# thenumbernine/lua-multigrid-poisson

Measured on AMD Instinct MI355X. Metric: V-cycles/sec + finest-smoother achieved HBM GB/s, 3D Poisson, higher is better.
Workload: dtype f32; 1 GPU; BASELINE configs[2]: 3D Poisson 512^3 per GPU, 7-point, RB-GS 2+2, V-cycle, trilinear P, 2x2x2-average R, consistent coarse boundary, per-cycle RMS-update err; parallelism=single GPU, levels=10

## Files before the change

lua-multigrid-poisson_amd/csrc/mgp_kernels.hip:

```cpp
#include "mgp_cell.h"
#include "mgp_zs.h"

#include <cstdio>
#include <cstdlib>
#include <type_traits>
#include <utility>

namespace mgp {
namespace {




template <typename T>
__global__ __launch_bounds__(kBlock) void k_init(T* __restrict__ u, T* __restrict__ f, Geo g, int64_t cx, int64_t cy,
                                                 int64_t cz, int dim3)
{
    const int64_t n = g.P * g.nz;
    for (int64_t s = (int64_t)blockIdx.x * kBlock + threadIdx.x; s < n; s += (int64_t)gridDim.x * kBlock) {
        int i, j;
        int64_t k;
        const bool cell = slot_cell(s, g, i, j, k);
        const double charge = 1e+6, epsilon0 = 1;
        const bool hit = cell && i == cx && j == cy && (!dim3 || g.z0 + k == cz);
// ... 890 lines not shown
            const T a01 = w0 * c01[pe] + w1 * nb01;
            const T a11 = w0 * c11[pe] + w1 * nb11;
            const T b0 = w0 * a00 + w1 * a10;
            const T b1 = w0 * a01 + w1 * a11;
            return w0 * b0 + w1 * b1;
        }
        const bool ox = (o == 0 && I0 + e == 0) || (o == 1 && I0 + e == cx - 1);
        if (!oy && !oz) {
            const T sx = -cl;
            auto nx_ = [&](const T (&cc)[N + 2]) {
                return ox ? (sx == (T)1 ? cc[pe] : sx * cc[pe]) : (o ? cc[e + 2] : cc[e]);
            };
            const T a00 = w0 * c00[pe] + w1 * nx_(c00);
            const T a10 = w0 * c10[pe] + w1 * nx_(c10);
            if (DIM == 2) return w0 * a00 + w1 * a10;
            const T a01 = w0 * c01[pe] + w1 * nx_(c01);
            const T a11 = w0 * c11[pe] + w1 * nx_(c11);
            const T b0 = w0 * a00 + w1 * a10;
            const T b1 = w0 * a01 + w1 * a11;
            return w0 * b0 + w1 * b1;
        }
        auto sv = [&](T val, bool fx, bool fy, bool fz) {
            T s = (T)1;
            if (fx) s = -cl * s;
            if (fy) s = -cl * s;
            if (fz) s = -cl * s;
            return s == (T)1 ? val : s * val;
        };
        auto col = [&](const T (&cc)[N + 2]) { return ox ? cc[pe] : (o ? cc[e + 2] : cc[e]); };
        const T a00 = w0 * c00[pe] + w1 * sv(col(c00), ox, false, false);
        const T a10 = w0 * sv(c10[pe], false, oy, false) + w1 * sv(col(c10), ox, oy, false);
        if (DIM == 2) return w0 * a00 + w1 * a10;
        const T a01 = w0 * sv(c01[pe], false, false, oz) + w1 * sv(col(c01), ox, false, oz);
        const T a11 = w0 * sv(c11[pe], false, oy, oz) + w1 * sv(col(c11), ox, oy, oz);
        const T b0 = w0 * a00 + w1 * a10;
        const T b1 = w0 * a01 + w1 * a11;
        return w0 * b0 + w1 * b1;
    }
};

template <typename T, int DIM, int LINEAR, bool BLACK = false>
__global__ __launch_bounds__(kBlock) void k_prolong_v(T* __restrict__ u, const T* __restrict__ V, Geo g, Geo gc,
                                                      T cl)
{
    constexpr int N = VN<T>::n;
    constexpr int LN = N == 4 ? 2 : 1;
    const int lgpr = gc.lx - LN;
    const int b = xcd_remap(blockIdx.x, gridDim.x);
    const int64_t it = (int64_t)b * kBlock + threadIdx.x;
    const int grp = (int)(it & ((1 << lgpr) - 1));
    const int j = (int)((it >> lgpr) & (g.ny - 1));
    const int64_t k = it >> (lgpr + g.ly);
    if (k >= (DIM == 3 ? (int64_t)g.nz : 1)) return;
    const int I0 = grp * N;
    PvRow<T, N, DIM, LINEAR> pv;
    pv.load(V, gc, j, k, I0);
    const int p = (int)((j + g.z0 + k) & 1);
#pragma unroll
    for (int c = BLACK ? 1 : 0; c < 2; ++c) {
        const int o = c ^ p;
        const int64_t own = k * g.P + c * g.H + (int64_t)j * g.hw + I0;
        Vec<T, N> uv = vload<T, N>(u + own);
#pragma unroll
        for (int e = 0; e < N; ++e) uv.v[e] = uv.v[e] + pv.value(e, o, cl);
        vstore<T, N>(u + own, uv);
    }
}

template <typename T, int DIM, int LINEAR>
__global__ __launch_bounds__(kBlock) void k_post1(T* __restrict__ u, const T* __restrict__ V,
                                                  const T* __restrict__ f, Geo g, Geo gc, Op<T, DIM> op, T clc)
{
    constexpr int N = VN<T>::n;
    constexpr int LN = N == 4 ? 2 : 1;
    const int lgpr = g.lhw - LN;
    const int b = xcd_remap(blockIdx.x, gridDim.x);
    const int64_t it = (int64_t)b * kBlock + threadIdx.x;
    const int grp = (int)(it & ((1 << lgpr) - 1));
    const int j = (int)((it >> lgpr) & (g.ny - 1));
    const int64_t k = it >> (lgpr + g.ly);
    if (k >= g.nz) return;
    const int m0 = grp * N;
    const int64_t gk = g.z0 + k;
    const int orr = (int)((j + gk) & 1);
    auto black_row = [&](int jj, int64_t kk, Vec<T, N>& r) {
        const int64_t gkk = g.z0 + kk;
        if (jj < 0 || jj >= g.ny || (DIM == 3 && (gkk < 0 || gkk >= g.gnz))) {
            r = vzero<T, N>();
            return;
        }
        const int ob = 1 ^ (int)((jj + gkk) & 1);
        r = vload<T, N>(u + kk * g.P + g.H + (int64_t)jj * g.hw + m0);
        PvRow<T, N, DIM, LINEAR> pv;
        pv.load(V, gc, jj, kk, m0);
#pragma unroll
        for (int e = 0; e < N; ++e) r.v[e] = r.v[e] + pv.value(e, ob, clc);
    };
    Vec<T, N> bc, byl, byr, bzl, bzr;
    black_row(j, k, bc);
    black_row(j - 1, k, byl);
    black_row(j + 1, k, byr);
    if (DIM == 3) {
        black_row(j, k - 1, bzl);
        black_row(j, k + 1, bzr);
    }
    const int me = orr == 0 ? m0 - 1 : m0 + N;
    T edge = (T)0;
    if (me >= 0 && me < g.hw) {
        const int i = 2 * me + (orr ^ 1);
        edge = u[k * g.P + g.H + (int64_t)j * g.hw + me] + prolong_value<T, DIM, LINEAR>(V, g, gc, clc, i, j, k);
    }
    const int64_t own = k * g.P + (int64_t)j * g.hw + m0;
    const Vec<T, N> fr = vload<T, N>(f + own);
    const int nbyz = (j == 0) + (j == g.ny - 1) + (DIM == 3 ? (gk == 0) + (gk == g.gnz - 1) : 0);
    Vec<T, N> out;
#pragma unroll
    for (int e = 0; e < N; ++e) {
        const int i = 2 * (m0 + e) + orr;
        const T xl = orr == 0 ? (e == 0 ? edge : bc.v[e - 1]) : bc.v[e];
        const T xr = orr == 0 ? bc.v[e] : (e == N - 1 ? edge : bc.v[e + 1]);
        T s = xl + xr;
        s = s + byl.v[e];
        s = s + byr.v[e];
        if (DIM == 3) {
            s = s + bzl.v[e];
            s = s + bzr.v[e];
        }
        out.v[e] = op.relax(s, fr.v[e], nbyz + (i == 0) + (i == g.nx - 1));
    }
    vstore<T, N>(u + own, out);
}


template <typename T>
struct ZsSplit {
    using S = ZsShape<T, true, true>;
    static_assert(S::XPAIR && S::H == 5 && S::NS3 == 4 && kZsRask, "the split follows k_zs's 64 x 32 PRE layout");
    static constexpr int NTW = S::TC / 64;
    static constexpr int NW = 2 * NTW + 4, NTL = 64 * NW, WMIX = NW - 1;
    static constexpr int MA = S::YT2 - S::YT2S, MB = 2 * S::G;
    static_assert(NTW == 4 && S::NTL == 64 * 7 && S::YT2S == 64 * 6 && S::YT0 == 64 * 5 && MA + MB <= 64, "wave order");
    static constexpr int wave_kind(int w) { return w == WMIX ? 2 : (w < 2 * NTW ? w >= NTW : ((w - 2 * NTW) & 1)); }
    static constexpr int local_wave(int w) { return w < 2 * NTW ? w % NTW : NTW + (w - 2 * NTW) / 2; }
    static constexpr int BT1 = S::YT0 + MB;
    static __device__ __forceinline__ int b_yrow(int t)
    {
        if (t < S::YT0) return S::yrow(t);
        if (t < BT1) return t - S::YT0 < S::G ? S::H - 1 : S::H + S::TY;
        return -1;
    }
    static __device__ __forceinline__ int b_ycol(int t) { return t < S::YT0 ? S::ycol(t) : (t - S::YT0) % S::G; }
    static constexpr int FROWS = S::TY + 2, FSLOT = FROWS * S::HWE;
    static constexpr int OFFFR = (int)(S::lds_bytes / sizeof(T)), OFFFB = OFFFR + 4 * FSLOT;
    static constexpr size_t lds_bytes = (size_t)(OFFFB + 4 * FSLOT) * sizeof(T);
    static_assert(NTL <= 1024 && NW <= 12, "too many waves for 168 VGPRs");
    static_assert(lds_bytes <= 160 * 1024, "LDS");
};

template <typename T, bool ZSRC, bool CLZ>
__device__ __forceinline__ void zs_split_body(const T* __restrict__ src, const T* __restrict__ f, T* __restrict__ dst,
                                              T* __restrict__ R, const Geo& g, const Geo& gc, const Op<T, 3>& op, int zc,
                                              int gz, int patch)
{
    using SP = ZsSplit<T>;
    static_assert(CLZ || (ZsShape<T, true, false>::TX == SP::S::TX && ZsShape<T, true, false>::TY == SP::S::TY &&
                          ZsShape<T, true, false>::N == SP::S::N),
                  "the split's cl != 0 levels run the cl = 0 tile");
    using S = typename SP::S;
    constexpr int N = S::N, H = S::H, HWE = S::HWE, G = S::G, YE = S::YE, SLOT = S::SLOT, TX = S::TX, TY = S::TY,
                  NS3 = S::NS3;
    using VT = Vec<T, N>;
    using PF = ZsPrefetch<T, N>;
    constexpr int PFD = ZS_PFD_PRE, NPF = PFD + 1, UNR = NPF == 3 ? 12 : 4;
    static_assert(PFD >= 1 && PFD <= 3, "prefetch distance 1..3");
    extern __shared__ __align__(16) unsigned char zs_smem[];
    T* const lds = reinterpret_cast<T*>(zs_smem);
    const int tid = threadIdx.x;

    const int tiles_x = g.nx / TX, tiles_y = g.ny / TY;
    const int b = xcd_remap(blockIdx.x, gridDim.x);
    const int tile = b % (tiles_x * tiles_y);
    const int Z0 = (b / (tiles_x * tiles_y)) * zc;
    int tx_, ty_;
    zs_tile_xy(tile, tiles_x, patch, tx_, ty_);
    const int X0 = tx_ * TX, Y0 = ty_ * TY;
    const int hw = g.hw, Hh = (int)g.H;
    const int z0 = (int)g.z0, gnz = (int)g.gnz, cz0 = (int)gc.z0;
    const int64_t P = g.P;
    const int qlo = -gz, qhi = (int)g.nz - 1 + gz;

    const int wv = __builtin_amdgcn_readfirstlane(tid >> 6), lane = tid & 63;
    const int wk = SP::wave_kind(wv), lw = SP::local_wave(wv);
    const bool grp_b = wk == 1 || (wk == 2 && lane >= SP::MA);
    const int lt = wk == 2 ? (grp_b ? S::YT0 + lane - SP::MA : S::YT2S + lane) : 64 * lw + lane;
    const int yr_ = grp_b ? SP::b_yrow(lt) : S::yrow(lt);
    const bool on = yr_ >= 0;
    const int gx = on ? (grp_b ? SP::b_ycol(lt) : S::ycol(lt)) : 0, ye = on ? yr_ : 0;
    const int gy = Y0 - H + ye;
    const int m0 = gx * N;
    ZsCol col;
    col.lrow = ye * HWE + m0;
    col.lym = (ye > 0 ? ye - 1 : ye) * HWE + m0;
    col.lyp = (ye < YE - 1 ? ye + 1 : ye) * HWE + m0;
    col.gm = (X0 - S::HX) / 2 + m0;
    col.x_first = gx == 0;
    col.x_last = gx == G - 1;
    col.lxm = col.x_first ? col.lrow : col.lrow - N;
    col.lxp = col.x_last ? col.lrow : col.lrow + N;
    const bool in_xy = on && gy >= 0 && gy < g.ny && col.gm >= 0 && col.gm < hw;
    col.xin = true;
    const int cgy = gy < 0 ? 0 : (gy >= g.ny ? g.ny - 1 : gy);
    const int cgm = col.gm < 0 ? 0 : (col.gm > hw - N ? hw - N : col.gm);
    const int goff = cgy * hw + cgm;
    const bool tile_xy = on && ye >= H && ye < H + TY && gx >= S::HXG && gx < G - S::HXG;
    const bool frow = on && ye >= H - 1 && ye <= H + TY;
    const int lf = frow ? (ye - (H - 1)) * HWE + m0 : 0;
    auto fslot = [&](int off, int q) { return lds + off + (q & 3) * SP::FSLOT + lf; };
    const int zlo = Z0 - H;
    ZsDiag<T> dz = {};
    if constexpr (!CLZ) {
        const int nby = (gy == 0) + (gy == g.ny - 1);
        dz.db = nby == 0 ? op.dg[0] : (nby == 1 ? op.dg[1] : op.dg[2]);
        dz.yb = nby == 0 ? op.ydg[0] : (nby == 1 ? op.ydg[1] : op.ydg[2]);
        dz.de = nby == 0 ? op.dg[1] : (nby == 1 ? op.dg[2] : op.dg[3]);
        dz.ye = nby == 0 ? op.ydg[1] : (nby == 1 ? op.ydg[2] : op.ydg[3]);
        dz.left = col.gm == 0;
        dz.right = col.gm + N == hw;
    }
    auto nbyz = [&](int q) {
        return CLZ ? 0 : (gy == 0) + (gy == g.ny - 1) + (z0 + q == 0) + (z0 + q == gnz - 1);
    };
    const int p_end = Z0 + zc + 6;
    auto inz = [&](int q) { return z0 + q >= 0 && z0 + q < gnz; };
    auto pcl = [&](int q) { return q < qlo ? qlo : (q > qhi ? qhi : q); };
    auto slot = [&](int off, int ns, int q) { return lds + off + (q & (ns - 1)) * SLOT; };
    const int rowpar = (gy + z0) & 1;
    auto par = [&](int q) { return rowpar ^ (q & 1); };
    const VT vz = vzero<T, N>();

    for (int i = tid; i < (int)(SP::lds_bytes / sizeof(T)); i += SP::NTL) lds[i] = (T)0;
    __syncthreads();

    constexpr bool PART = !CLZ;
    int ps = zlo, pe = p_end;
    ps = ps > 7 - z0 ? ps : 7 - z0;
    ps = ps > qlo + 4 ? ps : qlo + 4;
    pe = pe < gnz - 1 - z0 ? pe : gnz - 1 - z0;
    pe = pe < qhi - PFD ? pe : qhi - PFD;
    ps += (UNR - (ps - zlo) % UNR) % UNR;
    if (!PART) pe -= (pe - ps + 1) % UNR;
    if (pe < ps || ((z0 | Z0) & 1)) ps = pe = zlo - 1;
    const std::false_type GEN;
    const std::true_type STY;
    auto run = [&](auto&& prefetch, auto&& step) __attribute__((always_inline)) {
        PF pb[NPF];
#pragma unroll
        for (int k = 0; k < PFD; ++k) prefetch(GEN, pb[k], zlo + k);
        int p = zlo;
        auto group = [&](auto st, int p0, int pfirst, int plim) __attribute__((always_inline)) {
            zs_unroll<UNR>([&](auto kk) __attribute__((always_inline)) {
                constexpr int k = decltype(kk)::value;
                if (p0 + k >= pfirst && p0 + k <= plim) {
                    step(st, std::integral_constant<int, (k & 3)>(), pb[k % NPF], pb[(k + PFD) % NPF], p0 + k);
                    lds_barrier();
                }
            });
        };
        for (; p < ps; p += UNR) group(GEN, p, p, p + UNR);
        for (; p + UNR - 1 <= pe; p += UNR) group(STY, p, p, p + UNR);
        int pf = p;
        if constexpr (PART) {
            if (p <= pe) {
                group(STY, p, p, pe);
                pf = pe + 1;
            }
        }
        for (; p <= p_end; p += UNR) group(GEN, p, PART ? pf : p, p_end);
    };

    const T* const src_black = ZSRC ? nullptr : src + Hh;
    auto prefetch_a = [&](auto st, PF& r, int p) __attribute__((always_inline)) {
        constexpr bool ST = decltype(st)::value;
        if (ST) {
            const int64_t pP = (int64_t)p * P;
            if constexpr (ZSRC)
                r.u = vzero<T, N>();
            else
                r.u = gload<T, N, kZsNTL>(src_black + pP + goff);
            r.f1 = gload<T, N, kZsNTL>(f + (pP - P) + goff);
            r.f2 = gload<T, N, kZsNTL>(f + (pP - 2 * P) + Hh + goff);
        } else {
            if constexpr (ZSRC)
                r.u = vzero<T, N>();
            else
                r.u = gload<T, N, kZsNTL>(src_black + (int64_t)pcl(p) * P + goff);
            r.f1 = gload<T, N, kZsNTL>(f + (int64_t)pcl(p - 1) * P + goff);
            r.f2 = gload<T, N, kZsNTL>(f + (int64_t)pcl(p - 2) * P + Hh + goff);
        }
    };
    VT W0[4], W1[4], W2[4], FR[4];
#pragma unroll
    for (int i = 0; i < 4; ++i) W0[i] = W1[i] = W2[i] = FR[i] = vz;
    auto step_a = [&](auto st, auto rt, const PF& cur, PF& nxt, int p, int ro) __attribute__((always_inline)) {
        constexpr bool ST = decltype(st)::value;
        constexpr int RS = decltype(rt)::value;
        auto sl = [](int k) constexpr { return (RS - k) & 3; };
        if (ST) p = (p & ~1) | ((H + RS) & 1);
        zs_hold<T, N>(cur.u);
        zs_hold<T, N>(cur.f1);
        zs_hold<T, N>(cur.f2);
        asm volatile("" ::: "memory");
        if (ST || p + PFD <= p_end) prefetch_a(st, nxt, p + PFD);
        ZsNb<T, N> n1, n2, n3;
        VT a0 = cur.u;
        if (!ST && !inz(p)) a0 = vz;
        W0[sl(0)] = a0;
        zs_nb_load<T, N>(n1, slot(0, 2, p - 1), col);
        VT o1 = zs_relax<T, N, CLZ, ST, !CLZ>(W0[sl(2)], W0[sl(1)], W0[sl(0)], n1, cur.f1, col, par(p - 1), nbyz(p - 1), g.nx, op, dz);
        if (!ST && !inz(p - 1)) o1 = vz;
        W1[sl(1)] = o1;
        VT o2 = vz, o3 = vz;
        if (ro < 2) {
            zs_nb_load<T, N>(n2, slot(S::OFF1, 2, p - 2), col);
            o2 = zs_relax<T, N, CLZ, ST, !CLZ>(W1[sl(3)], W1[sl(2)], W1[sl(1)], n2, cur.f2, col, 1 ^ par(p - 2), nbyz(p - 2), g.nx, op, dz);
            if (!ST && !inz(p - 2)) o2 = vz;
            W2[sl(2)] = o2;
            zs_nb_load<T, N>(n3, slot(S::OFF2, 2, p - 3), col);
            o3 = zs_relax<T, N, CLZ, ST, !CLZ>(W2[sl(4)], W2[sl(3)], W2[sl(2)], n3, FR[sl(3)], col, par(p - 3), nbyz(p - 3), g.nx, op, dz);
            if (!ST && !inz(p - 3)) o3 = vz;
        }
        if (in_xy) {
            vstore<T, N>(slot(0, 2, p) + col.lrow, a0);
            vstore<T, N>(slot(S::OFF1, 2, p - 1) + col.lrow, o1);
            if (ro < 2) {
                vstore<T, N>(slot(S::OFF2, 2, p - 2) + col.lrow, o2);
                vstore<T, N>(slot(S::OFF3, NS3, p - 3) + col.lrow, o3);
            }
            if (frow) {
                vstore<T, N>(fslot(SP::OFFFR, p - 3), FR[sl(3)]);
                vstore<T, N>(fslot(SP::OFFFB, p - 2), cur.f2);
            }
        }
        FR[sl(1)] = cur.f1;
    };

    auto prefetch_b = [](auto, PF&, int) {};
    VT W3[4], W4[4], FB[4];
    T AS[2][N], acc[N];
#pragma unroll
    for (int e = 0; e < N; ++e) AS[0][e] = AS[1][e] = acc[e] = (T)0;
#pragma unroll
    for (int i = 0; i < 4; ++i) W3[i] = W4[i] = FB[i] = vz;
    const bool even_row = (gy & 1) == 0;
    T* const xbase = lds + S::OFFX + (((ye + (H & 1)) >> 1) * G + gx) * 2 * N;
    auto xs = [&](int q) { return xbase + (q & 1) * (S::XPAIRS * G * 2 * N); };
    auto step_b = [&](auto st, auto rt, auto tw, int p) __attribute__((always_inline)) {
        constexpr bool ST = decltype(st)::value;
        constexpr int RS = decltype(rt)::value;
        auto sl = [](int k) constexpr { return (RS - k) & 3; };
        if (ST) p = (p & ~1) | ((H + RS) & 1);
        const int zz0 = ST ? (z0 & ~1) : z0;
        ZsNb<T, N> n4, nk;
        const VT fb = vload<T, N>(fslot(SP::OFFFB, p - 5));
        W3[sl(4)] = vload<T, N>(slot(S::OFF3, NS3, p - 4) + col.lrow);
        zs_nb_load<T, N>(n4, slot(S::OFF3, NS3, p - 5), col);
        VT o4 = zs_relax_a<T, N, CLZ, ST, !CLZ>(W3[sl(6)], W3[sl(5)], W3[sl(4)], n4, fb, col, 1 ^ par(p - 5), nbyz(p - 5), g.nx, op, dz,
                                           AS[RS & 1]);
        if (!ST && !inz(p - 5)) o4 = vz;
        W4[sl(5)] = o4;
        if (in_xy) vstore<T, N>(slot(S::OFF4, 2, p - 5) + col.lrow, o4);
        if constexpr (decltype(tw)::value) {
            {
                const int q = p - 5;
                if (q >= Z0 && q < Z0 + zc && tile_xy) gstore<T, N, kZsNTS>(dst + (int64_t)q * P + Hh + goff, o4);
            }
            const int q = p - 6;
            const int pq = par(q);
            zs_nb_load<T, N>(nk, slot(S::OFF4, 2, q), col);
            T xr[2 * N];
            {
                const T* x = xs(q - 1);
#pragma unroll
                for (int e = 0; e < 2 * N; ++e) xr[e] = x[e];
            }
            T rred[N], rblk[N], rr[2][N];
            const VT fr = vload<T, N>(fslot(SP::OFFFR, q));
            zs_residual<T, N, CLZ, ST, !CLZ>(W4[sl(7)], W4[sl(6)], W4[sl(5)], nk, W3[sl(6)], fr, col, pq, nbyz(q), g.nx, op, dz, rred);
            zs_residual_a<T, N, CLZ, ST, !CLZ>(AS[(RS & 1) ^ 1], W4[sl(6)], FB[sl(6)], col, 1 ^ pq, nbyz(q), g.nx, op, dz, rblk);
#pragma unroll
            for (int e = 0; e < N; ++e) {
                rr[0][e] = pq == 0 ? rred[e] : rblk[e];
                rr[1][e] = pq == 0 ? rblk[e] : rred[e];
            }
            const int dq = q - (ST ? (Z0 & ~1) : Z0);
            if (dq >= 0 && dq <= zc && tile_xy)
                zs_restrict_avg<T, N>(rr, xr, acc, dq, zc, even_row, xs(q), R, (zz0 + q - 1) >> 1, gy >> 1, col.gm, cz0, gc);
            FB[sl(5)] = fb;
        }
    };

    if (wk == 0) {
        const int wrole = S::wave_role(lw);
        run(prefetch_a, [&](auto st, auto rt, const PF& cur, PF& nxt, int p) __attribute__((always_inline)) {
            step_a(st, rt, cur, nxt, p, decltype(st)::value ? wrole : 0);
        });
    } else if (wk == 1) {
        if (lw < SP::NTW)
            run(prefetch_b, [&](auto st, auto rt, const PF& cur, PF& nxt, int p) __attribute__((always_inline)) {
                step_b(st, rt, STY, p);
            });
        else
            run(prefetch_b, [&](auto st, auto rt, const PF& cur, PF& nxt, int p) __attribute__((always_inline)) {
                step_b(st, rt, GEN, p);
            });
    } else {
        run(
            [&](auto st, PF& r, int p) __attribute__((always_inline)) {
                if (!grp_b) prefetch_a(st, r, p);
            },
            [&](auto st, auto rt, const PF& cur, PF& nxt, int p) __attribute__((always_inline)) {
                if (!grp_b) step_a(st, rt, cur, nxt, p, 2);
                asm volatile("" ::: "memory");
                if (grp_b) step_b(st, rt, GEN, p);
            });
    }
}

template <typename T, bool ZSRC>
__global__ __launch_bounds__((ZsSplit<T>::NTL)) void k_zs_split(const T* __restrict__ src, const T* __restrict__ f,
                                                                 T* __restrict__ dst, T* __restrict__ R, Geo g, Geo gc,
                                                                 Op<T, 3> op, int zc, int gz, int patch)
{
    zs_split_body<T, ZSRC, true>(src, f, dst, R, g, gc, op, zc, gz, patch);
}

template <typename T>
__global__ __launch_bounds__((ZsSplit<T>::NTL)) void k_zs_split_cl(const T* __restrict__ f, T* __restrict__ dst,
                                                                    T* __restrict__ R, Geo g, Geo gc, Op<T, 3> op, int zc,
                                                                    int gz, int patch)
{
    zs_split_body<T, true, false>(nullptr, f, dst, R, g, gc, op, zc, gz, patch);
}

template <typename T>
struct ZsSplitPost {
    using S = ZsShape<T, false, true, true, false, 4>;
    static_assert(S::N == 4 && S::H == 4 && S::HXG == 1 && S::NS3 == 2 && !S::PS && !S::YROLE, "POST's wide tile, 16-byte columns");
    static constexpr int G = S::G, NA = S::NT, NA2 = G * (S::TY + 4), NA3 = NA2 + 2 * G;
    static constexpr int BROWS = S::TY + 2, GC = G - 2 * S::HXG, NBT = G * S::TY, NB = NBT + 2 * GC;
    static constexpr int NWA = NA / 64, NWB = NB / 64, MA = NA - 64 * NWA;
    static constexpr int NW = NWA + NWB + 1, NTL = 64 * NW, WLAST = NW - 1;
    static constexpr unsigned BMASK = 0x25A;
    static_assert(NWA == 6 && NWB == 5 && NB == 64 * NWB && MA > 0 && NW == 12, "wave order");
    static __device__ __forceinline__ int wave_kind(int w) { return w == WLAST ? 2 : (int)((BMASK >> w) & 1u); }
    static __device__ __forceinline__ int local_wave(int w)
    {
        const unsigned below = (1u << w) - 1u;
        return __builtin_popcount(((BMASK >> w) & 1u) ? (BMASK & below) : (~BMASK & below));
    }
    static_assert(NA2 <= 64 * NWA, "A's last wave holds rows d >= 3 only");
    static __device__ __forceinline__ int a_yrow(int t)
    {
        if (t < NA2) return 2 + t / G;
        if (t < NA3) return t - NA2 < G ? 1 : S::YE - 2;
        if (t < NA) return t - NA3 < G ? 0 : S::YE - 1;
        return -1;
    }
    static __device__ __forceinline__ int b_yrow(int t)
    {
        if (t < NBT) return S::H + t / G;
        return t - NBT < GC ? S::H - 1 : S::H + S::TY;
    }
    static __device__ __forceinline__ int b_ycol(int t) { return t < NBT ? t % G : S::HXG + (t - NBT) % GC; }
    static constexpr int SLOT = S::SLOT, OFF1 = 2 * SLOT, OFF2 = 4 * SLOT, OFF3 = 8 * SLOT, OFFC = 10 * SLOT;
    static constexpr int FSLOT = BROWS * S::HWE;
    static constexpr int OFFFR = OFFC + 4 * S::CSLOT, OFFFB = OFFFR + 4 * FSLOT;
    static constexpr size_t lds_bytes = (size_t)(OFFFB + 4 * FSLOT) * sizeof(T);
    static constexpr int EG = (S::TX + 8) / 4, ENT = (EG * S::YE + 63) / 64 * 64;
    static_assert(OFFC % 4 == 0 && S::CPAIRS <= 2 * NB, "coarse staging: two pairs per thread of B");
    static_assert(NTL <= 1024 && NW <= 12, "too many waves for 168 VGPRs");
    static_assert(lds_bytes + ENT * sizeof(double) <= 160 * 1024, "LDS");
    static_assert(ENT <= 1024 && ENT - 512 <= NTL, "the sum's first level within the workgroup");
};

template <typename T, bool ERR>
__global__ __launch_bounds__((ZsSplitPost<T>::NTL)) void k_zs_split_post(const T* __restrict__ src, const T* __restrict__ f,
                                                                          T* __restrict__ dst, const T* old,
                                                                          const T* __restrict__ V,
                                                                          double* __restrict__ partials, Geo g, Geo gc,
                                                                          Op<T, 3> op, T clc, int zc, int gz, int patch)
{
    using SP = ZsSplitPost<T>;
    using S = typename SP::S;
    constexpr int N = S::N, H = S::H, HWE = S::HWE, G = S::G, YE = S::YE, SLOT = S::SLOT, TX = S::TX, TY = S::TY;
    using VT = Vec<T, N>;
    using PF = ZsPrefetch<T, N>;
    constexpr int PFD = 1, NPF = PFD + 1, UNR = 4;
    extern __shared__ __align__(16) unsigned char zs_smem[];
    T* const lds = reinterpret_cast<T*>(zs_smem);
    const int tid = threadIdx.x;

    const int tiles_x = g.nx / TX, tiles_y = g.ny / TY;
    const int b = xcd_remap(blockIdx.x, gridDim.x);
    const int tile = b % (tiles_x * tiles_y);
    const int Z0 = (b / (tiles_x * tiles_y)) * zc;
    int tx_, ty_;
    zs_tile_xy(tile, tiles_x, patch, tx_, ty_);
    const int X0 = tx_ * TX, Y0 = ty_ * TY;
    const int hw = g.hw, Hh = (int)g.H;
    const int z0 = (int)g.z0, gnz = (int)g.gnz, cz0 = (int)gc.z0;
    const int64_t P = g.P;
    const int qlo = -gz, qhi = (int)g.nz - 1 + gz;

    const int wv = __builtin_amdgcn_readfirstlane(tid >> 6), lane = tid & 63;
    const int wk = SP::wave_kind(wv), lw = SP::local_wave(wv);
    const bool grp_b = wk == 1;
    const int lt = wk == 2 ? 64 * SP::NWA + lane : 64 * lw + lane;
    const int yr_ = grp_b ? SP::b_yrow(lt) : SP::a_yrow(lt);
    const bool on = yr_ >= 0;
    const int gx = on ? (grp_b ? SP::b_ycol(lt) : lt % G) : 0, ye = on ? yr_ : 0;
    const int gy = Y0 - H + ye;
    const int m0 = gx * N;
    ZsCol col;
    col.lrow = ye * HWE + m0;
    col.lym = (ye > 0 ? ye - 1 : ye) * HWE + m0;
    col.lyp = (ye < YE - 1 ? ye + 1 : ye) * HWE + m0;
    col.gm = (X0 - S::HX) / 2 + m0;
    col.x_first = gx == 0;
    col.x_last = gx == G - 1;
    col.lxm = col.x_first ? col.lrow : col.lrow - N;
    col.lxp = col.x_last ? col.lrow : col.lrow + N;
    const bool in_xy = on && gy >= 0 && gy < g.ny && col.gm >= 0 && col.gm < hw;
    col.xin = true;
    const int cgy = gy < 0 ? 0 : (gy >= g.ny ? g.ny - 1 : gy);
    const int cgm = col.gm < 0 ? 0 : (col.gm > hw - N ? hw - N : col.gm);
    const int goff = cgy * hw + cgm;
    const bool tile_xy = on && ye >= H && ye < H + TY && gx >= S::HXG && gx < G - S::HXG;
    const int ydist = ye < H ? H - ye : (ye >= H + TY ? ye - (H + TY) + 1 : 0);
    const bool need_f1 = !ZS_FHALO || ydist <= H - 1, need_f2 = !ZS_FHALO || ydist <= H - 2;
    const bool frow = on && ye >= H - 1 && ye <= H + TY;
    const int lf = frow ? (ye - (H - 1)) * HWE + m0 : 0;
    auto fslot = [&](int off, int q) { return lds + off + (q & 3) * SP::FSLOT + lf; };
    const int zlo = Z0 - H;
    const ZsDiag<T> dz = {};
    const int p_end = Z0 + zc + 4;
    auto inz = [&](int q) { return z0 + q >= 0 && z0 + q < gnz; };
    auto pcl = [&](int q) { return q < qlo ? qlo : (q > qhi ? qhi : q); };
    auto slot = [&](int off, int ns, int q) { return lds + off + (q & (ns - 1)) * SLOT; };
    const int rowpar = (gy + z0) & 1;
// ... 1420 lines not shown
```

lua-multigrid-poisson_amd/csrc/mgp_zs.h:

```cpp
#pragma once
#include "mgp_device.h"

#include <cstdio>
#include <type_traits>
#include <utility>

namespace mgp {
namespace {


#ifdef ZS_NOCHAIN
#define ZS_NC 1
#else
#define ZS_NC 0
#endif
#ifdef ZS_NOLOAD
#define ZS_PLANE(q) 0
#else
#define ZS_PLANE(q) (q)
#endif

#ifndef ZS_NPRE_F32
#define ZS_NPRE_F32 4
#endif
// ... 355 lines not shown
            const bool edge = (e == 0 && o == 0 && dz.left) || (e == N - 1 && o == 1 && dz.right);
            const T a_u = ask[e] + (edge ? de : db) * uc.v[e];
            rr[e] = fv.v[e] - a_u;
        }
    } else if (CLZ || __all(nbyz == 0 && c.xin)) {
#pragma unroll
        for (int e = 0; e < N; ++e) {
            const T a_u = ask[e] + op.adiag * uc.v[e];
            rr[e] = fv.v[e] - a_u;
        }
    } else {
#pragma unroll
        for (int e = 0; e < N; ++e) {
            const int i = 2 * (c.gm + e) + o;
            const T a_u = ask[e] + op.diag_direct(nbyz + (i == 0) + (i == nx - 1)) * uc.v[e];
            rr[e] = fv.v[e] - a_u;
        }
    }
}

template <typename T, int N>
struct ZsCoarse {
    T c00[N + 2], c10[N + 2], c01[N + 2], c11[N + 2];
};

template <typename T, int N, int LINEAR>
__device__ __forceinline__ void zs_correct(Vec<T, N>& uv, const ZsCoarse<T, N>& cur, int o, int I0, int cx, bool oy,
                                           bool oz, T cl, bool fast)
{
    const T w0 = (T)0.75, w1 = (T)0.25;
    if (!LINEAR) {
#pragma unroll
        for (int e = 0; e < N; ++e) uv.v[e] = uv.v[e] + cur.c00[e + 1];
        return;
    }
    if (fast) {
#pragma unroll
        for (int e = 0; e < N; ++e) {
            const int pe = e + 1;
            const T nb00 = o ? cur.c00[e + 2] : cur.c00[e];
            const T nb10 = o ? cur.c10[e + 2] : cur.c10[e];
            const T nb01 = o ? cur.c01[e + 2] : cur.c01[e];
            const T nb11 = o ? cur.c11[e + 2] : cur.c11[e];
            const T a00 = w0 * cur.c00[pe] + w1 * nb00;
            const T a10 = w0 * cur.c10[pe] + w1 * nb10;
            const T a01 = w0 * cur.c01[pe] + w1 * nb01;
            const T a11 = w0 * cur.c11[pe] + w1 * nb11;
            const T b0 = w0 * a00 + w1 * a10;
            const T b1 = w0 * a01 + w1 * a11;
            uv.v[e] = uv.v[e] + (w0 * b0 + w1 * b1);
        }
        return;
    }
    auto sv = [&](T val, bool fx, bool fy, bool fz) {
        T s = (T)1;
        if (fx) s = -cl * s;
        if (fy) s = -cl * s;
        if (fz) s = -cl * s;
        return s == (T)1 ? val : s * val;
    };
#pragma unroll
    for (int e = 0; e < N; ++e) {
        const int pe = e + 1;
        const bool ox = (o == 0 && I0 + e == 0) || (o == 1 && I0 + e == cx - 1);
        auto col = [&](const T (&cc)[N + 2]) { return ox ? cc[pe] : (o ? cc[e + 2] : cc[e]); };
        const T a00 = w0 * cur.c00[pe] + w1 * sv(col(cur.c00), ox, false, false);
        const T a10 = w0 * sv(cur.c10[pe], false, oy, false) + w1 * sv(col(cur.c10), ox, oy, false);
        const T a01 = w0 * sv(cur.c01[pe], false, false, oz) + w1 * sv(col(cur.c01), ox, false, oz);
        const T a11 = w0 * sv(cur.c11[pe], false, oy, oz) + w1 * sv(col(cur.c11), ox, oy, oz);
        const T b0 = w0 * a00 + w1 * a10;
        const T b1 = w0 * a01 + w1 * a11;
        uv.v[e] = uv.v[e] + (w0 * b0 + w1 * b1);
    }
}

template <typename T, int N>
__device__ __forceinline__ void zs_bq(T (&b)[N], const T (&c0)[N + 2], const T (&c1)[N + 2], int o, int I0, int cx,
                                      bool oy, T cl, bool fast)
{
    const T w0 = (T)0.75, w1 = (T)0.25;
    if (fast) {
#pragma unroll
        for (int e = 0; e < N; ++e) {
            const T nb0 = o ? c0[e + 2] : c0[e];
            const T nb1 = o ? c1[e + 2] : c1[e];
            const T a0 = w0 * c0[e + 1] + w1 * nb0;
            const T a1 = w0 * c1[e + 1] + w1 * nb1;
            b[e] = w0 * a0 + w1 * a1;
        }
        return;
    }
    auto sv = [&](T val, bool fx, bool fy) {
        T s = (T)1;
        if (fx) s = -cl * s;
        if (fy) s = -cl * s;
        return s == (T)1 ? val : s * val;
    };
#pragma unroll
    for (int e = 0; e < N; ++e) {
        const int pe = e + 1;
        const bool ox = (o == 0 && I0 + e == 0) || (o == 1 && I0 + e == cx - 1);
        auto col = [&](const T (&cc)[N + 2]) { return ox ? cc[pe] : (o ? cc[e + 2] : cc[e]); };
        const T a0 = w0 * c0[pe] + w1 * sv(col(c0), ox, false);
        const T a1 = w0 * sv(c1[pe], false, oy) + w1 * sv(col(c1), ox, oy);
        b[e] = w0 * a0 + w1 * a1;
    }
}


#ifndef ZS_WPE_PRE
#define ZS_WPE_PRE 2
#endif
#ifndef ZS_PFD_PRE
#define ZS_PFD_PRE 2
#endif
#ifndef ZS_PFD_POST
#define ZS_PFD_POST 1
#endif
#ifndef ZS_PFD_PRE_CL
#define ZS_PFD_PRE_CL 1
#endif
template <typename F, int... K>
__device__ __forceinline__ void zs_unroll_impl(F& f, std::integer_sequence<int, K...>)
{
    (f(std::integral_constant<int, K>()), ...);
}
template <int U, typename F>
__device__ __forceinline__ void zs_unroll(F&& f)
{
    zs_unroll_impl(f, std::make_integer_sequence<int, U>());
}
#ifndef ZS_BQ
#define ZS_BQ 1
#endif
#ifndef ZS_RASK
#define ZS_RASK 1
#endif
constexpr bool kZsRask = ZS_RASK != 0;
#ifndef ZS_WPE_POST
#define ZS_WPE_POST 4
#endif
__device__ __forceinline__ void zs_tile_xy(int tile, int tiles_x, int patch, int& tx, int& ty)
{
    tx = tile % tiles_x;
    ty = tile / tiles_x;
    if (patch) {
        const int px = patch & 255, py = patch >> 8, per = px * py, prow = tiles_x / px;
        const int pi = tile / per, q = tile % per;
        tx = (pi % prow) * px + q % px;
        ty = (pi / prow) * py + q / px;
    }
}

template <typename T, int N>
__device__ __forceinline__ void zs_restrict_avg(const T (&rr)[2][N], const T (&xr)[2 * N], T (&acc)[N], int dq, int zc,
                                                bool even_row, T* xw, T* __restrict__ R, int K, int J, int gm, int cz0,
                                                const Geo& gc)
{
    if (!even_row) {
        if (dq < zc) {
#pragma unroll
            for (int e = 0; e < N; ++e) {
                xw[e] = rr[0][e];
                xw[N + e] = rr[1][e];
            }
        }
    } else {
        if (dq >= 1) {
#pragma unroll
            for (int e = 0; e < N; ++e) {
                acc[e] = acc[e] + xr[e];
                acc[e] = acc[e] + xr[N + e];
            }
            if ((dq & 1) == 0) {
                T* rowc = R + (int64_t)(K - cz0) * gc.P + (int64_t)J * gc.hw;
#pragma unroll
                for (int e = 0; e < N; ++e) {
                    const int I = gm + e;
                    rowc[((I + J + K) & 1) * gc.H + (I >> 1)] = (T)0.125 * acc[e];
                }
            }
        }
        if (dq < zc) {
#pragma unroll
            for (int e = 0; e < N; ++e) {
                if ((dq & 1) == 0) {
                    acc[e] = rr[0][e] + rr[1][e];
                } else {
                    acc[e] = acc[e] + rr[0][e];
                    acc[e] = acc[e] + rr[1][e];
                }
            }
        }
    }
}

template <typename T, bool PRE, int LINEAR, bool ERR, bool CLZ, bool WIDE = false>
__global__ __launch_bounds__((ZsShape<T, PRE, CLZ, WIDE, PRE && LINEAR == 2>::NTL))
__attribute__((amdgpu_waves_per_eu(1, PRE ? ZS_WPE_PRE : ZS_WPE_POST))) void k_zs(const T* __restrict__ src, const T* __restrict__ f,
                                                                T* __restrict__ dst, const T* old, T* __restrict__ R,
                                                                const T* __restrict__ V, double* __restrict__ partials,
                                                                Geo g, Geo gc, Op<T, 3> op, T clc, int zc, int gz,
                                                                int patch)
{
    constexpr bool FWF = PRE && LINEAR == 2;
    using S = ZsShape<T, PRE, CLZ, WIDE, FWF>;
    constexpr int N = S::N, H = S::H, HWE = S::HWE, G = S::G, YE = S::YE, SLOT = S::SLOT, TX = S::TX,
                  TY = S::TY, NS3 = S::NS3, NTL = S::NTL;
    constexpr bool RR = PRE && LINEAR == 0;
    constexpr bool ZSRC = PRE && ERR;
    using VT = Vec<T, N>;
    using PF = ZsPrefetch<T, N>;
    constexpr int PFD = PRE ? (CLZ ? ZS_PFD_PRE : ZS_PFD_PRE_CL) : ZS_PFD_POST, NPF = PFD + 1, UNR = NPF == 3 ? 12 : 4;
    static_assert(PFD >= 1 && PFD <= 3, "prefetch distance 1..3");
    extern __shared__ __align__(16) unsigned char zs_smem[];
    T* const lds = reinterpret_cast<T*>(zs_smem);
    const int tid = threadIdx.x;

    const int tiles_x = g.nx / TX, tiles_y = g.ny / TY;
    const int b = xcd_remap(blockIdx.x, gridDim.x);
    const int tile = b % (tiles_x * tiles_y);
    const int Z0 = (b / (tiles_x * tiles_y)) * zc;
    int tx_, ty_;
    zs_tile_xy(tile, tiles_x, patch, tx_, ty_);
    const int X0 = tx_ * TX, Y0 = ty_ * TY;
    const int hw = g.hw, Hh = (int)g.H;
    const int z0 = (int)g.z0, gnz = (int)g.gnz, cz0 = (int)gc.z0;
    const int64_t P = g.P;
    const int qlo = -gz, qhi = (int)g.nz - 1 + gz;

    const int wcls = S::PS ? __builtin_amdgcn_readfirstlane(tid >= S::NPAR ? 1 : 0) : 0;
    const int rt_ = S::PS ? tid - wcls * S::NPAR : tid;
    const int yr_ = S::PS ? 0 : S::yrow(tid);
    const bool on = S::PS ? rt_ < G * (wcls ? YE / 2 : S::YEV) : yr_ >= 0;
    const int gx = on ? (S::PS ? rt_ % G : S::ycol(tid)) : 0, ye = S::PS ? (on ? 2 * (rt_ / G) + wcls : wcls) : (on ? yr_ : 0);
    const int gy = Y0 - H + ye;
    const int m0 = gx * N;
    ZsCol col;
    auto lr = [&](int y) { return S::PS ? (y & 1) * S::YEV + (y >> 1) : y; };
    col.lrow = lr(ye) * HWE + m0;
    col.lym = lr(ye > 0 ? ye - 1 : ye) * HWE + m0;
    col.lyp = lr(ye < YE - 1 ? ye + 1 : ye) * HWE + m0;
    col.gm = (X0 - S::HX) / 2 + m0;
    col.x_first = gx == 0;
    col.x_last = gx == G - 1;
    col.lxm = col.x_first ? col.lrow : col.lrow - N;
    col.lxp = col.x_last ? col.lrow : col.lrow + N;
    const bool in_xy = on && gy >= 0 && gy < g.ny && col.gm >= 0 && col.gm < hw;
    col.xin = !in_xy || (col.gm > 0 && 2 * (col.gm + N) < g.nx);
    const int cgy = gy < 0 ? 0 : (gy >= g.ny ? g.ny - 1 : gy);
    const int cgm = col.gm < 0 ? 0 : (col.gm > hw - N ? hw - N : col.gm);
#if defined(ZS_HALO_ALIAS)
    const int agm = (ZS_HALO_ALIAS & 1) ? (gx < S::HXG ? cgm + S::HXG * N : (gx >= G - S::HXG ? cgm - S::HXG * N : cgm)) : cgm;
    const int agy = (ZS_HALO_ALIAS & 2) ? (ye < H ? cgy + H : (ye >= H + TY ? cgy - H : cgy)) : cgy;
    const int goff = agy * hw + agm;
#else
    const int goff = cgy * hw + cgm;
#endif
    const bool tile_xy = on && ye >= H && ye < H + TY && gx >= S::HXG && gx < G - S::HXG;
    const int ydist = ye < H ? H - ye : (ye >= H + TY ? ye - (H + TY) + 1 : 0);
    const bool need_f1 = !ZS_FHALO || PRE || ydist <= H - 1, need_f2 = !ZS_FHALO || PRE || ydist <= H - 2;
    const int zlo = Z0 - H;
    ZsDiag<T> dz;
    {
        const int nby = (gy == 0) + (gy == g.ny - 1);
        dz.db = nby == 0 ? op.dg[0] : (nby == 1 ? op.dg[1] : op.dg[2]);
        dz.yb = nby == 0 ? op.ydg[0] : (nby == 1 ? op.ydg[1] : op.ydg[2]);
        dz.de = nby == 0 ? op.dg[1] : (nby == 1 ? op.dg[2] : op.dg[3]);
        dz.ye = nby == 0 ? op.ydg[1] : (nby == 1 ? op.ydg[2] : op.ydg[3]);
        dz.left = col.gm == 0;
        dz.right = col.gm + N == hw;
    }
    const int p_end = Z0 + zc + (PRE ? (FWF ? 7 : 5) : 3);
    auto inz = [&](int q) { return z0 + q >= 0 && z0 + q < gnz; };
    auto pcl = [&](int q) { return q < qlo ? qlo : (q > qhi ? qhi : q); };
    auto slot = [&](int off, int ns, int q) {
        const int r = ns == 3 ? ((q % 3) + 3) % 3 : (q & (ns - 1));
        return lds + off + r * SLOT;
    };
    auto nbyz = [&](int q) {
        return CLZ ? 0 : (gy == 0) + (gy == g.ny - 1) + (z0 + q == 0) + (z0 + q == gnz - 1);
    };
    const int rowpar = (gy + z0) & 1;
    const int wrole = S::YROLE ? __builtin_amdgcn_readfirstlane(S::wave_role(tid >> 6)) : 0;
    const T* const src_black = ZSRC ? nullptr : src + Hh;

    for (int i = tid; i < (int)(S::lds_bytes / sizeof(T)); i += NTL) lds[i] = (T)0;
    __syncthreads();

    const int Ia = X0 / 2 - 8, Ja = Y0 / 2 - 3;
    auto ckl = [&](int K) { return K < 0 ? 0 : (K >= gc.gnz ? gc.gnz - 1 : K); };
    auto cslot = [&](int K) { return lds + S::OFFC + (K & 3) * S::CSLOT; };
    auto cload = [&](PF& r, int K) {
        K = ckl(K);
#pragma unroll
        for (int i = 0; i < 2; ++i) {
            const int t = tid + i * NTL;
            const int J = Ja + t / (S::CI / 2), I = Ia + 2 * (t % (S::CI / 2));
            r.cv[i].v[0] = r.cv[i].v[1] = (T)0;
            if (t < S::CPAIRS && J >= 0 && J < gc.ny && I >= 0 && I < gc.nx) {
                const T* row = V + (int64_t)(K - cz0) * gc.P + (int64_t)J * gc.hw + (I >> 1);
                const int ce = (I + J + K) & 1;
                r.cv[i].v[0] = row[ce * gc.H];
                r.cv[i].v[1] = row[(ce ^ 1) * gc.H];
            }
        }
    };
    auto cstore = [&](const PF& r, int K) {
        T* const sl = cslot(ckl(K));
#pragma unroll
        for (int i = 0; i < 2; ++i) {
            const int t = tid + i * NTL;
            if (t < S::CPAIRS) vstore<T, 2>(sl + 2 * t, r.cv[i]);
// ... 513 lines not shown
```

Before: 1101 V-cycles/s (512^3-cell slabs, whole job).

## Hoist LDS neighbour reads and make LDS stores unconditional via sink slot

In the split zs smoother kernel, neighbour LDS reads are issued earlier (before prefetch and preceding relax steps) and split into a read phase and a pick phase, separated by sched_barriers. Conditional LDS stores become branch-free by redirecting inactive lanes to a dedicated sink region, and the restriction x-pair write is moved out of zs_restrict_avg into the same predicated-store path. The aim is to overlap LDS latency with compute and remove divergent store branches. The cost is extra LDS footprint for the sink and more live registers, which could reduce occupancy.

```diff
diff --git a/lua-multigrid-poisson_amd/csrc/mgp_kernels.hip b/lua-multigrid-poisson_amd/csrc/mgp_kernels.hip
--- a/lua-multigrid-poisson_amd/csrc/mgp_kernels.hip
+++ b/lua-multigrid-poisson_amd/csrc/mgp_kernels.hip
@@ -1066,7 +1066,14 @@
     static __device__ __forceinline__ int b_ycol(int t) { return t < S::YT0 ? S::ycol(t) : (t - S::YT0) % S::G; }
     static constexpr int FROWS = S::TY + 2, FSLOT = FROWS * S::HWE;
     static constexpr int OFFFR = (int)(S::lds_bytes / sizeof(T)), OFFFB = OFFFR + 4 * FSLOT;
-    static constexpr size_t lds_bytes = (size_t)(OFFFB + 4 * FSLOT) * sizeof(T);
+    static_assert(S::lds_bytes % 16 == 0, "16-byte f cells");
+    static constexpr int NSA = 2, NSF = 4;
+    static constexpr int OFFSINK = OFFFB + NSF * FSLOT;
+    static constexpr int XHALF = S::XPAIRS * S::G * 2 * S::N, SINKN = XHALF > S::SLOT ? XHALF : S::SLOT;
+    static_assert(FSLOT <= SINKN, "the sink holds a slot of every ring");
+    static constexpr size_t lds_bytes = (size_t)(OFFSINK + SINKN) * sizeof(T);
+    static constexpr bool ring_apart(int ns, int w, int r) { return (r - w) % ns != 0; }
+    static_assert(OFFSINK % S::N == 0, "16-byte sink cells");
     static_assert(NTL <= 1024 && NW <= 12, "too many waves for 168 VGPRs");
     static_assert(lds_bytes <= 160 * 1024, "LDS");
 };
@@ -1130,6 +1137,36 @@
     const bool frow = on && ye >= H - 1 && ye <= H + TY;
     const int lf = frow ? (ye - (H - 1)) * HWE + m0 : 0;
     auto fslot = [&](int off, int q) { return lds + off + (q & 3) * SP::FSLOT + lf; };
+    const bool f_xy = in_xy && frow;
+    auto put = [&](bool mine, int base, int rel, const VT& v) __attribute__((always_inline)) {
+#ifndef ZS_NOLDSWRITE
+        vstore<T, N>(lds + (mine ? base : SP::OFFSINK) + rel, v);
+#endif
+    };
+    auto slot_at = [&](int off, int ns, int q) { return off + (q & (ns - 1)) * SLOT; };
+    auto fslot_at = [&](int off, int q) { return off + (q & (SP::NSF - 1)) * SP::FSLOT; };
+    struct NbX {
+        VT l, r;
+    };
+    auto nb_read = [&](ZsNb<T, N>& nb, NbX& w, const T* s_in) __attribute__((always_inline)) {
+#ifdef ZS_NOLDSREAD
+        zs_nb_load<T, N>(nb, s_in, col);
+        w.l = w.r = vzero<T, N>();
+        return;
+#endif
+        nb.yl = vload<T, N>(s_in + col.lym);
+        nb.yr = vload<T, N>(s_in + col.lyp);
+        w.l = vload_lds_whole<T, N>(s_in + col.lxm);
+        w.r = vload_lds_whole<T, N>(s_in + col.lxp);
+    };
+    auto nb_pick = [&](ZsNb<T, N>& nb, const NbX& w) __attribute__((always_inline)) {
+#ifndef ZS_NOLDSREAD
+        zs_hold<T, N>(w.l);
+        zs_hold<T, N>(w.r);
+        nb.ep = (col.x_first && !ZS_XRAW) ? (T)0 : w.l.v[N - 1];
+        nb.en = (col.x_last && !ZS_XRAW) ? (T)0 : w.r.v[0];
+#endif
+    };
     const int zlo = Z0 - H;
     ZsDiag<T> dz = {};
     if constexpr (!CLZ) {
@@ -1220,40 +1257,42 @@
         constexpr int RS = decltype(rt)::value;
         auto sl = [](int k) constexpr { return (RS - k) & 3; };
         if (ST) p = (p & ~1) | ((H + RS) & 1);
+        ZsNb<T, N> n1, n2, n3;
+        NbX x1, x2, x3;
+        nb_read(n1, x1, slot(0, SP::NSA, p - 1));
+        if (ro < 2) nb_read(n2, x2, slot(S::OFF1, SP::NSA, p - 2));
         zs_hold<T, N>(cur.u);
         zs_hold<T, N>(cur.f1);
         zs_hold<T, N>(cur.f2);
         asm volatile("" ::: "memory");
         if (ST || p + PFD <= p_end) prefetch_a(st, nxt, p + PFD);
-        ZsNb<T, N> n1, n2, n3;
+        static_assert(SP::ring_apart(SP::NSA, 0, 1) && SP::ring_apart(SP::NSA, 1, 2) && SP::ring_apart(SP::NSA, 2, 3), "A's rings");
+        static_assert(SP::ring_apart(NS3, 3, 4) && SP::ring_apart(NS3, 3, 5), "the hand-off ring");
+        static_assert(SP::ring_apart(SP::NSF, 3, 6) && SP::ring_apart(SP::NSF, 2, 5), "the f rings");
         VT a0 = cur.u;
         if (!ST && !inz(p)) a0 = vz;
         W0[sl(0)] = a0;
-        zs_nb_load<T, N>(n1, slot(0, 2, p - 1), col);
+        put(in_xy, slot_at(0, SP::NSA, p), col.lrow, a0);
+        put(f_xy, fslot_at(SP::OFFFR, p - 3), lf, FR[sl(3)]);
+        put(f_xy, fslot_at(SP::OFFFB, p - 2), lf, cur.f2);
+        nb_pick(n1, x1);
         VT o1 = zs_relax<T, N, CLZ, ST, !CLZ>(W0[sl(2)], W0[sl(1)], W0[sl(0)], n1, cur.f1, col, par(p - 1), nbyz(p - 1), g.nx, op, dz);
         if (!ST && !inz(p - 1)) o1 = vz;
         W1[sl(1)] = o1;
-        VT o2 = vz, o3 = vz;
+        put(in_xy, slot_at(S::OFF1, SP::NSA, p - 1), col.lrow, o1);
         if (ro < 2) {
-            zs_nb_load<T, N>(n2, slot(S::OFF1, 2, p - 2), col);
-            o2 = zs_relax<T, N, CLZ, ST, !CLZ>(W1[sl(3)], W1[sl(2)], W1[sl(1)], n2, cur.f2, col, 1 ^ par(p - 2), nbyz(p - 2), g.nx, op, dz);
+            nb_read(n3, x3, slot(S::OFF2, SP::NSA, p - 3));
+            __builtin_amdgcn_sched_barrier(0);
+            nb_pick(n2, x2);
+            VT o2 = zs_relax<T, N, CLZ, ST, !CLZ>(W1[sl(3)], W1[sl(2)], W1[sl(1)], n2, cur.f2, col, 1 ^ par(p - 2), nbyz(p - 2), g.nx, op, dz);
             if (!ST && !inz(p - 2)) o2 = vz;
             W2[sl(2)] = o2;
-            zs_nb_load<T, N>(n3, slot(S::OFF2, 2, p - 3), col);
-            o3 = zs_relax<T, N, CLZ, ST, !CLZ>(W2[sl(4)], W2[sl(3)], W2[sl(2)], n3, FR[sl(3)], col, par(p - 3), nbyz(p - 3), g.nx, op, dz);
+            put(in_xy, slot_at(S::OFF2, SP::NSA, p - 2), col.lrow, o2);
+            __builtin_amdgcn_sched_barrier(0);
+            nb_pick(n3, x3);
+            VT o3 = zs_relax<T, N, CLZ, ST, !CLZ>(W2[sl(4)], W2[sl(3)], W2[sl(2)], n3, FR[sl(3)], col, par(p - 3), nbyz(p - 3), g.nx, op, dz);
             if (!ST && !inz(p - 3)) o3 = vz;
-        }
-        if (in_xy) {
-            vstore<T, N>(slot(0, 2, p) + col.lrow, a0);
-            vstore<T, N>(slot(S::OFF1, 2, p - 1) + col.lrow, o1);
-            if (ro < 2) {
-                vstore<T, N>(slot(S::OFF2, 2, p - 2) + col.lrow, o2);
-                vstore<T, N>(slot(S::OFF3, NS3, p - 3) + col.lrow, o3);
-            }
-            if (frow) {
-                vstore<T, N>(fslot(SP::OFFFR, p - 3), FR[sl(3)]);
-                vstore<T, N>(fslot(SP::OFFFB, p - 2), cur.f2);
-            }
+            put(in_xy, slot_at(S::OFF3, NS3, p - 3), col.lrow, o3);
         }
         FR[sl(1)] = cur.f1;
     };
@@ -1266,7 +1305,8 @@
 #pragma unroll
     for (int i = 0; i < 4; ++i) W3[i] = W4[i] = FB[i] = vz;
     const bool even_row = (gy & 1) == 0;
-    T* const xbase = lds + S::OFFX + (((ye + (H & 1)) >> 1) * G + gx) * 2 * N;
+    const int xrel = ((((ye + (H & 1)) >> 1) * G + gx) * 2 * N);
+    T* const xbase = lds + S::OFFX + xrel;
     auto xs = [&](int q) { return xbase + (q & 1) * (S::XPAIRS * G * 2 * N); };
     auto step_b = [&](auto st, auto rt, auto tw, int p) __attribute__((always_inline)) {
         constexpr bool ST = decltype(st)::value;
@@ -1275,30 +1315,35 @@
         if (ST) p = (p & ~1) | ((H + RS) & 1);
         const int zz0 = ST ? (z0 & ~1) : z0;
         ZsNb<T, N> n4, nk;
+        NbX x4, xk;
         const VT fb = vload<T, N>(fslot(SP::OFFFB, p - 5));
         W3[sl(4)] = vload<T, N>(slot(S::OFF3, NS3, p - 4) + col.lrow);
-        zs_nb_load<T, N>(n4, slot(S::OFF3, NS3, p - 5), col);
+        nb_read(n4, x4, slot(S::OFF3, NS3, p - 5));
+        const int q = p - 6;
+        T xr[2 * N];
+        if constexpr (decltype(tw)::value) {
+            nb_read(nk, xk, slot(S::OFF4, SP::NSA, q));
+            const T* x = xs(q - 1);
+#pragma unroll
+            for (int e = 0; e < 2 * N; ++e) xr[e] = x[e];
+        }
+        __builtin_amdgcn_sched_barrier(0);
+        static_assert(SP::ring_apart(SP::NSA, 5, 6) && SP::ring_apart(2, 0, 1), "B's rings");
+        nb_pick(n4, x4);
         VT o4 = zs_relax_a<T, N, CLZ, ST, !CLZ>(W3[sl(6)], W3[sl(5)], W3[sl(4)], n4, fb, col, 1 ^ par(p - 5), nbyz(p - 5), g.nx, op, dz,
                                            AS[RS & 1]);
         if (!ST && !inz(p - 5)) o4 = vz;
         W4[sl(5)] = o4;
-        if (in_xy) vstore<T, N>(slot(S::OFF4, 2, p - 5) + col.lrow, o4);
+        put(in_xy, slot_at(S::OFF4, SP::NSA, p - 5), col.lrow, o4);
         if constexpr (decltype(tw)::value) {
             {
-                const int q = p - 5;
-                if (q >= Z0 && q < Z0 + zc && tile_xy) gstore<T, N, kZsNTS>(dst + (int64_t)q * P + Hh + goff, o4);
+                const int q5 = p - 5;
+                if (q5 >= Z0 && q5 < Z0 + zc && tile_xy) gstore<T, N, kZsNTS>(dst + (int64_t)q5 * P + Hh + goff, o4);
             }
-            const int q = p - 6;
             const int pq = par(q);
-            zs_nb_load<T, N>(nk, slot(S::OFF4, 2, q), col);
-            T xr[2 * N];
-            {
-                const T* x = xs(q - 1);
-#pragma unroll
-                for (int e = 0; e < 2 * N; ++e) xr[e] = x[e];
-            }
             T rred[N], rblk[N], rr[2][N];
             const VT fr = vload<T, N>(fslot(SP::OFFFR, q));
+            nb_pick(nk, xk);
             zs_residual<T, N, CLZ, ST, !CLZ>(W4[sl(7)], W4[sl(6)], W4[sl(5)], nk, W3[sl(6)], fr, col, pq, nbyz(q), g.nx, op, dz, rred);
             zs_residual_a<T, N, CLZ, ST, !CLZ>(AS[(RS & 1) ^ 1], W4[sl(6)], FB[sl(6)], col, 1 ^ pq, nbyz(q), g.nx, op, dz, rblk);
 #pragma unroll
@@ -1307,8 +1352,20 @@
                 rr[1][e] = pq == 0 ? rblk[e] : rred[e];
             }
             const int dq = q - (ST ? (Z0 & ~1) : Z0);
+            {
+                const bool mine = dq >= 0 && dq < zc && tile_xy && !even_row;
+                VT r0, r1;
+#pragma unroll
+                for (int e = 0; e < N; ++e) {
+                    r0.v[e] = rr[0][e];
+                    r1.v[e] = rr[1][e];
+                }
+                const int xw = S::OFFX + (q & 1) * SP::XHALF;
+                vstore<T, N>(lds + (mine ? xw : SP::OFFSINK) + xrel, r0);
+                vstore<T, N>(lds + (mine ? xw : SP::OFFSINK) + xrel + N, r1);
+            }
             if (dq >= 0 && dq <= zc && tile_xy)
-                zs_restrict_avg<T, N>(rr, xr, acc, dq, zc, even_row, xs(q), R, (zz0 + q - 1) >> 1, gy >> 1, col.gm, cz0, gc);
+                zs_restrict_avg<T, N, false>(rr, xr, acc, dq, zc, even_row, nullptr, R, (zz0 + q - 1) >> 1, gy >> 1, col.gm, cz0, gc);
             FB[sl(5)] = fb;
         }
     };
diff --git a/lua-multigrid-poisson_amd/csrc/mgp_zs.h b/lua-multigrid-poisson_amd/csrc/mgp_zs.h
--- a/lua-multigrid-poisson_amd/csrc/mgp_zs.h
+++ b/lua-multigrid-poisson_amd/csrc/mgp_zs.h
@@ -531,13 +531,13 @@
     }
 }
 
-template <typename T, int N>
+template <typename T, int N, bool XW = true>
 __device__ __forceinline__ void zs_restrict_avg(const T (&rr)[2][N], const T (&xr)[2 * N], T (&acc)[N], int dq, int zc,
                                                 bool even_row, T* xw, T* __restrict__ R, int K, int J, int gm, int cz0,
                                                 const Geo& gc)
 {
     if (!even_row) {
-        if (dq < zc) {
+        if (XW && dq < zc) {
 #pragma unroll
             for (int e = 0; e < N; ++e) {
                 xw[e] = rr[0][e];
```

After: 1112 V-cycles/s (512^3-cell slabs, whole job) (median of 6 runs). About the same (+1.0%).
